# keeffEoghan/tendrils

Hardware: AMD Instinct MI355X
Metric: particle-steps/sec (16M particles per GPU) (higher is better)
Workload: dtype f32

## Files before the change

include/tendrils_hip.h:

```cpp
#ifndef TENDRILS_HIP_H
#define TENDRILS_HIP_H

#include <stddef.h>
#include <stdint.h>

#ifdef __cplusplus
extern "C" {
#endif

#define TH_ABI_VERSION 14

typedef int32_t th_status;
enum {
    TH_OK = 0,
    TH_ERR_INVALID = 1,
    TH_ERR_HIP = 2,
    TH_ERR_NO_DEVICE = 3,
    TH_ERR_UNSUPPORTED = 4
};

#define TH_INERT (-1000000.0f)

typedef struct th_context th_context;

// ... 295 lines not shown
    uint64_t fragments, crowded_fragments;
    uint64_t sent_bytes, received_bytes;
} th_draw_info;
th_status th_draw_query(th_context *ctx, th_draw_info *out);

typedef struct th_flow_line_uniforms {
    float speed, rad, crestShape, speedLimit;
    float viewSize[2];
} th_flow_line_uniforms;

th_status th_flow_line_attributes(const float *points, const double *times, int32_t n, int32_t closed, int32_t capacity,
                                  int32_t *nverts, float *position, float *normal, float *miter, float *previous,
                                  float *time, float *dt);
th_status th_flow_lines(th_context *ctx, const th_flow_line_uniforms *u, const float *points, const double *times,
                        const int32_t *offsets, const int32_t *closed, int32_t nlines);

enum { TH_OPT_BUCKET = 0, TH_OPT_RESORT_STEPS = 1, TH_OPT_REBUCKET_STEPS = 2, TH_OPT_FUSE = 3, TH_OPT_GRAPH = 4,
       TH_OPT_FORCE_GENERIC = 5, TH_OPT_DRAW_REUSE = 6, TH_OPT_BINS_POOL = 7,
#ifdef TH_TESTING
       TH_OPT_INJECT_FAILURE = 8,
#endif
       TH_OPT_BINS_PAGES = 9, TH_OPT_ASYNC_SORT = 10, TH_OPT_SKIP_UNSEEN = 11, TH_OPT_SPAWN_CHUNK_ROWS = 12,
       TH_OPT_HASH_WINDOW = 13, TH_OPT_HASH_WINDOW_LAUNCHES = 14, TH_OPT_DENSE_SORTS = 15,
       TH_OPT_STAGE_BINS = 16, TH_OPT_LINE_BINS = 17 };
th_status th_option_set(th_context *ctx, int32_t option, int64_t value);
th_status th_option_get(th_context *ctx, int32_t option, int64_t *value);

#ifdef __cplusplus
}
#endif
#endif
```

tendrils_amd/csrc/th_api.hip:

```cpp
#include "th_ctx.hpp"

using namespace thi;

namespace {

thread_local std::string g_error;

void build_gradient_table(float4 *lut)
{
    for (int a = th::kLutMin; a <= th::kLutMax; ++a) {
        float p = th::permute_ref((float)a);
        float gx, gy, gz;
        th::gradient_ref(p, gx, gy, gz);
        lut[a - th::kLutMin] = make_float4(gx, gy, gz, 0.0f);
    }
}

void options_from_environment(th_options &o)
{
    auto number = [](const char *name, long long otherwise) { const char *e = getenv(name); return e && *e ? atoll(e) : otherwise; };
    o.bucket = (int)number("TH_BUCKET", -1);
    o.resort_steps = (int)number("TH_RESORT_STEPS", 64); if (o.resort_steps <= 0) o.resort_steps = 64;
    o.rebucket_steps = (int)number("TH_REBUCKET_STEPS", 256); if (o.rebucket_steps <= 0) o.rebucket_steps = 256;
    o.fuse = number("TH_FUSE", 1) != 0;
// ... 521 lines not shown
    out->state_w = c->cfg.width; out->state_h = c->cfg.height;
    out->flow_w = c->fw; out->flow_h = c->fh;
    out->frames_w = c->frw; out->frames_h = c->frh;
    return TH_OK;
}

th_status th_option_set(th_context *c, int32_t option, int64_t value)
{
    if (th_status s = use(c)) return s;
    th_options &o = c->opt;
    switch (option) {
    case TH_OPT_BUCKET: TH_REQUIRE(value >= -1 && value <= 1, "TH_OPT_BUCKET takes -1, 0 or 1"); o.bucket = (int)value; break;
    case TH_OPT_RESORT_STEPS: TH_REQUIRE(value > 0 && value < (1 << 30), "TH_OPT_RESORT_STEPS must be positive"); o.resort_steps = (int)value; break;
    case TH_OPT_REBUCKET_STEPS: TH_REQUIRE(value > 0 && value < (1 << 30), "TH_OPT_REBUCKET_STEPS must be positive"); o.rebucket_steps = (int)value; break;
    case TH_OPT_FUSE: o.fuse = value != 0; break;
    case TH_OPT_GRAPH: o.graph = value != 0; break;
    case TH_OPT_FORCE_GENERIC: o.force_generic = value != 0; break;
    case TH_OPT_DRAW_REUSE: o.draw_reuse = value != 0; break;
    case TH_OPT_SKIP_UNSEEN: o.skip_unseen = value != 0; break;
    case TH_OPT_HASH_WINDOW: o.hash_window = value != 0; break;
    case TH_OPT_STAGE_BINS: o.stage_bins = value != 0; break;
    case TH_OPT_LINE_BINS: o.line_bins = value != 0; break;
    case TH_OPT_HASH_WINDOW_LAUNCHES: return fail(TH_ERR_INVALID, "TH_OPT_HASH_WINDOW_LAUNCHES is read-only");
    case TH_OPT_DENSE_SORTS: return fail(TH_ERR_INVALID, "TH_OPT_DENSE_SORTS is read-only");
    case TH_OPT_ASYNC_SORT: o.async_sort = value != 0; if (!o.async_sort) { if (th_status s = asort_drop(c)) return s; } break;
    case TH_OPT_BINS_POOL: TH_REQUIRE(value >= 0 && value < (1ll << 32), "TH_OPT_BINS_POOL out of range"); o.bins_pool = (uint32_t)value; break;
#ifdef TH_TESTING
    case TH_OPT_INJECT_FAILURE: TH_REQUIRE(value >= 0 && value <= 5, "TH_OPT_INJECT_FAILURE takes 0..5"); o.inject_failure = (int)value; break;
#endif
    case TH_OPT_SPAWN_CHUNK_ROWS: TH_REQUIRE(value >= 0 && value < (1 << 30), "TH_OPT_SPAWN_CHUNK_ROWS takes 0 (by the scratch budget) or a number of rows"); o.spawn_chunk_rows = (int)value; break;
    case TH_OPT_BINS_PAGES:
        TH_REQUIRE(value >= -(int64_t)th::kBinPagesLimit && value <= (int64_t)th::kBinPagesLimit && value != 1 && value != -1, "TH_OPT_BINS_PAGES takes 0, or 2..%u (negative: never widened)", th::kBinPagesLimit);
        o.bins_pages = (int)value;
        if (c->chunk_table) {
            TH_HIP(hipStreamSynchronize(c->stream));
            c->chunk_table.reset(); c->bin_mem.reset(); c->bin_capacity = 0; c->bin_max_pages = 0;
        }
        break;
    default: return fail(TH_ERR_INVALID, "unknown option %d", option);
    }
    clear_graphs(c);
    return TH_OK;
}

th_status th_option_get(th_context *c, int32_t option, int64_t *value)
{
    TH_REQUIRE(c && value, "null argument");
    const th_options &o = c->opt;
    switch (option) {
    case TH_OPT_BUCKET: *value = o.bucket; break;
    case TH_OPT_RESORT_STEPS: *value = o.resort_steps; break;
    case TH_OPT_REBUCKET_STEPS: *value = o.rebucket_steps; break;
    case TH_OPT_FUSE: *value = o.fuse; break;
    case TH_OPT_GRAPH: *value = o.graph; break;
    case TH_OPT_FORCE_GENERIC: *value = o.force_generic; break;
    case TH_OPT_DRAW_REUSE: *value = o.draw_reuse; break;
    case TH_OPT_ASYNC_SORT: *value = o.async_sort; break;
    case TH_OPT_SKIP_UNSEEN: *value = o.skip_unseen; break;
    case TH_OPT_HASH_WINDOW: *value = o.hash_window; break;
    case TH_OPT_STAGE_BINS: *value = o.stage_bins; break;
    case TH_OPT_LINE_BINS: *value = o.line_bins; break;
    case TH_OPT_HASH_WINDOW_LAUNCHES: *value = c->hash_window_launches; break;
    case TH_OPT_DENSE_SORTS: *value = c->dense_sorts; break;
    case TH_OPT_BINS_POOL: *value = o.bins_pool; break;
#ifdef TH_TESTING
    case TH_OPT_INJECT_FAILURE: *value = o.inject_failure; break;
#endif
    case TH_OPT_BINS_PAGES: *value = o.bins_pages; break;
    case TH_OPT_SPAWN_CHUNK_ROWS: *value = o.spawn_chunk_rows; break;
    default: return fail(TH_ERR_INVALID, "unknown option %d", option);
    }
    return TH_OK;
}

}
```

tendrils_amd/csrc/th_ctx.hpp:

```cpp
#pragma once
#include <hip/hip_runtime.h>

#include <algorithm>
#include <atomic>
#include <cmath>
#include <cstdarg>
#include <cstdio>
#include <cstdlib>
#include <cstring>
#include <limits>
#include <memory>
#include <mutex>
#include <new>
#include <string>
#include <vector>

#include "th_kernels.hpp"
#include "th_math.hpp"
#include "th_program_kinds.hpp"

namespace thi {
struct FlowLineScratch;
th_status fail(th_status code, const char *fmt, ...);
std::string &last_error();
// ... 84 lines not shown
    th::LogicParams key{};
    hipGraphExec_t exec = nullptr;
    DevBuf<float> times_dev;
    HostBuf<float> times_host;
    hipEvent_t copied = nullptr;
};

struct th_context {
    th_config cfg{};
    th_options opt{};
    hipStream_t stream = nullptr;
    std::vector<float4 *> ring;
    bool packed = false;
    DevBuf<float4> tmp[3];
    DevBuf<float4> flow;
    DevBuf<float2> flow_dec;
    DevBuf<float> flow3;
    int32_t fw = 0, fh = 0;
    DevBuf<float4> targets;
    bool targets_checked = true, targets_nonfinite = false;
    DevBuf<float4> lut_block;
    float4 *lut = nullptr;
    DevBuf<float4> win_block;
    long long dense_sorts = 0;
    long long hash_window_launches = 0;
    DevBuf<uchar4> frames[2];
    int32_t frw = 0, frh = 0;
    DevBuf<unsigned int> d_flag;
    DevBuf<th::StatsPartial> partials;
    DevBuf<th::StatsPartial> fused_parts;
    struct { bool valid = false; const float4 *buf = nullptr; float limit = 0.0f; uint32_t nparts = 0; } fused_stats;
    DevBuf<th_counters> d_counters;
    DevBuf<float4> x_halo;
    DevBuf<unsigned long long> x_counts;
    DevBuf<unsigned long long> x_keys;
    DevBuf<float4> x_colors;
    DevBuf<float4> gathered;
    const void *gathered_of = nullptr;
    DevBuf<char> sp_taps;
    DevBuf<uint32_t> sp_asked;
    DevBuf<float4> sp_answers;
    DevBuf<unsigned long long> sp_words;
    th_spawn_info last_spawn{};
    void *comm = nullptr;
    const th::Transport *transport = nullptr;
    DevBuf<uint32_t> d_status;
    DevBuf<uint32_t> own_mem;
    bool sharded_draw_ready = false;
// ... 302 lines not shown
```

tendrils_amd/csrc/th_kernels.hip:

```cpp
#include "th_kernels.hpp"
#include "th_math.hpp"
#include "th_logic.hpp"

#include <type_traits>
#include <cstdlib>

namespace th {


__global__ __launch_bounds__(256) void pack_state_kernel(uint2 *dst, const float4 *src, uint32_t n)
{
    for (uint32_t i = blockIdx.x * 256u + threadIdx.x; i < n; i += gridDim.x * 256u) dst[i] = pack_state(src[i]);
}

__global__ __launch_bounds__(256) void unpack_state_kernel(float4 *dst, const uint2 *src, uint32_t n)
{
    for (uint32_t i = blockIdx.x * 256u + threadIdx.x; i < n; i += gridDim.x * 256u) dst[i] = unpack_state(src[i]);
}

void launch_pack_state(void *dst, const float4 *src, uint32_t n, hipStream_t s)
{
    if (n) hipLaunchKernelGGL(pack_state_kernel, dim3(grid_for(n, 8)), dim3(256), 0, s, (uint2 *)dst, src, n);
}

void launch_unpack_state(float4 *dst, const void *src, uint32_t n, hipStream_t s)
{
    if (n) hipLaunchKernelGGL(unpack_state_kernel, dim3(grid_for(n, 8)), dim3(256), 0, s, dst, (const uint2 *)src, n);
}

__global__ __launch_bounds__(256) void hash_tables_kernel(float4 *block)
{
    uint32_t *a = reinterpret_cast<uint32_t *>(block), *b = a + kPermA;
    for (int k = threadIdx.x; k < kPermA; k += 256) a[k] = 4u * (uint32_t)permute_int((float)k) - kBiasBitsA;
    for (int k = threadIdx.x; k < kPermB; k += 256) b[k] = 16u * (uint32_t)((int)permute_int((float)k) - kLutMin) - kBiasBitsB;
}
void launch_hash_tables(float4 *block, hipStream_t s) { hipLaunchKernelGGL(hash_tables_kernel, dim3(1), dim3(256), 0, s, block); }
int hash_table_vectors() { return kHashVec; }

__global__ __launch_bounds__(256) void win_tables_kernel(float4 *block, const float4 *lut)
{
    uint32_t *a = reinterpret_cast<uint32_t *>(block), *b = a + kWinA;
    float4 *g = block + kWinVec;
    for (int k = threadIdx.x; k < kWinA; k += 256) a[k] = 4u * (uint32_t)permute_int((float)(k % 289)) - kBiasBitsA;
    for (int k = threadIdx.x; k < kWinB; k += 256) b[k] = 16u * (uint32_t)((int)permute_int((float)(k % 289)) - kLutMin) - kBiasBitsB;
    for (int k = threadIdx.x; k < kWinG; k += 256) g[k] = lut[k % 289 - kLutMin];
}
void launch_win_tables(float4 *block, const float4 *lut, hipStream_t s) { hipLaunchKernelGGL(win_tables_kernel, dim3(1), dim3(256), 0, s, block, lut); }
int win_table_vectors() { return kWinVec + kWinG; }



struct F32Texel {
    using Word = float4;
    static constexpr bool packed = false;
    TH_D static Word empty() { return make_float4(0.0f, 0.0f, 0.0f, 0.0f); }
    TH_D static Word load(const float4 *buf, uint32_t i) { return load_stream(&buf[i]); }
    TH_D static void store(float4 *buf, uint32_t i, Word w) { store_stream(&buf[i], w); }
    TH_D static float4 decode(Word w) { return w; }
    TH_D static Word encode(float4 s) { return s; }
    TH_D static float4 quantize(float4 s) { return s; }
};
struct PackedTexel {
    using Word = v2u;
    static constexpr bool packed = true;
    TH_D static Word empty() { return Word{0x80008000u, 0u}; }
    TH_D static Word load(const float4 *buf, uint32_t i) { return __builtin_nontemporal_load(&reinterpret_cast<const v2u *>(buf)[i]); }
    TH_D static void store(float4 *buf, uint32_t i, Word w) { __builtin_nontemporal_store(w, &reinterpret_cast<v2u *>(buf)[i]); }
    TH_D static float4 decode(Word w) { return unpack_state(make_uint2(w.x, w.y)); }
    TH_D static Word encode(float4 s) { const uint2 q = pack_state(s); return Word{q.x, q.y}; }
    TH_D static float4 quantize(float4 s) { return quantize_state(s); }
};
// ... 87 lines not shown
    double sum = fin ? (double)sp : 0.0;
    float mx = fin ? sp : 0.0f;
#pragma unroll
    for (int o = 32; o > 0; o >>= 1) {
        sum += __shfl_xor(sum, o);
        const float om = __shfl_xor(mx, o); mx = om > mx ? om : mx;
    }
    if (__lane_id() == (uint32_t)__builtin_ctzll(__ballot(true))) {
        t.sum_speed = sum; t.max_speed = (double)mx;
        if (!first) {
            const StatsPartial o = *slot;
            t.live += o.live; t.nan += o.nan; t.capped += o.capped; t.sum_speed += o.sum_speed;
            t.max_speed = o.max_speed > t.max_speed ? o.max_speed : t.max_speed;
        }
        *slot = t;
    }
}

TH_D void stats_none(StatsPartial *slot, bool first)
{
    if (__ballot(!first) == 0ull && __lane_id() == 0u) *slot = StatsPartial{0ull, 0ull, 0ull, 0.0, 0.0};
}

#define TH_LOGIC_FUSED_LOOP(Fmt)                                                                                              \
    static_assert(!WIN || (NOISE && !FAST), "WIN: NOISE, exact");                                                              \
    __shared__ float4 smem[WIN ? kWinVec + kWinG : NOISE ? kHashVec + kLutSize : 1];                                          \
    const float4 *lut = smem + (WIN ? kWinVec + kLutMin : NOISE ? kHashVec : 0);                                              \
    const HashTables tabs{reinterpret_cast<const uint32_t *>(smem), reinterpret_cast<const uint32_t *>(smem) + (WIN ? kWinA : kPermA)}; \
    if constexpr (NOISE) {                                                                                                    \
        if constexpr (WIN) fill_win_tables(smem, p.win);                                                                      \
        else fill_hash_tables(smem, p.lut);                                                                                   \
        __syncthreads();                                                                                                      \
    }                                                                                                                         \
    uint32_t idx, stride, end;                                                                                                \
    if constexpr (!BUCKETED) {                                                                                                \
        idx = blockIdx.x * 256u + threadIdx.x;                                                                                \
        stride = gridDim.x * 256u;                                                                                            \
        end = p.count;                                                                                                        \
    } else {                                                                                                                  \
        const uint32_t group = blockIdx.x & 7u, rank = blockIdx.x >> 3, per = (p.count + 7u) >> 3;                            \
        const uint32_t lo = group * per;                                                                                      \
        idx = lo + rank * 256u + threadIdx.x;                                                                                 \
        stride = (gridDim.x >> 3) * 256u;                                                                                     \
        end = lo + per < p.count ? lo + per : p.count;                                                                        \
    }                                                                                                                         \
    typename Fmt::Word nxt = Fmt::empty();                                                                                    \
    uint32_t npid = idx;                                                                                                      \
    [[maybe_unused]] bool first = true;                                                                                       \
    if (idx < end) {                                                                                                          \
        nxt = Fmt::load(p.in, idx);                                                                                           \
        if constexpr (BUCKETED) npid = __builtin_nontemporal_load(&p.perm[idx]);                                              \
    }                                                                                                                         \
    for (; idx < end; idx += stride) {                                                                                        \
        const typename Fmt::Word w = nxt;                                                                                     \
        const uint32_t pid = BUCKETED ? npid : idx;                                                                           \
        if (idx + stride < end) {                                                                                             \
            nxt = Fmt::load(p.in, idx + stride);                                                                              \
            if constexpr (BUCKETED) npid = __builtin_nontemporal_load(&p.perm[idx + stride]);                                 \
        }                                                                                                                     \
        float4 st = Fmt::decode(w);                                                                                           \
        uint32_t left = p.nsteps;                                                                                             \
        do {                                                                                                                  \
            if (left == 1u) {                                                                                                 \
                uint32_t at = idx;                                                                                            \
                asm volatile("" : "+v"(at));                                                                                  \
                if (Fmt::packed && p.nsteps == 1u) Fmt::store(p.out_prev, at, w);                                             \
                else Fmt::store(p.out_prev, at, Fmt::encode(st));                                                             \
            }                                                                                                                 \
            st = Fmt::quantize(integrate<FAST, NOISE, TARGET, POW2, false, true, !NOISE, WIN>(p, lut, st, pid, p.times[p.nsteps - left], &tabs)); \
        } while (--left);                                                                                                     \
        Fmt::store(p.out, idx, Fmt::encode(st));                                                                              \
        if constexpr (STATS) { stats_take(&p.stats_part[blockIdx.x * 4u + (threadIdx.x >> 6)], st, p.u.speedLimit, first); first = false; } \
    }                                                                                                                         \
    if constexpr (STATS) stats_none(&p.stats_part[blockIdx.x * 4u + (threadIdx.x >> 6)], first);

template <bool FAST, bool NOISE, bool TARGET, bool POW2, bool BUCKETED, bool STATS, bool WIN>
__global__ __launch_bounds__(256) void logic_fused_kernel(const LogicParams p) { TH_LOGIC_FUSED_LOOP(F32Texel) }

template <bool FAST, bool NOISE, bool TARGET, bool POW2, bool BUCKETED, bool STATS, bool WIN>
__global__ __launch_bounds__(256, 5) void logic_fused_packed_kernel(const LogicParams p) { TH_LOGIC_FUSED_LOOP(PackedTexel) }

int fused_grid(uint32_t count, bool bucketed)
{
    const uint32_t blocks = (count + 255u) / 256u;
    const uint32_t grid = bucketed ? 8u * ((((count + 7u) >> 3) + 255u) / 256u) : blocks;
    return (int)(grid ? grid : 1u);
}

void launch_logic_fused(const LogicParams &p, const LogicVariant &v, hipStream_t s)
{
    if (!p.nsteps) return;
    const bool packed = v.format == StateFormat::packed, bucketed = p.perm != nullptr;
    const int grid = fused_grid(p.count, bucketed);
    lift([&](auto fast, auto noise, auto target, auto pow2, auto bk, auto stats, auto window) {
        constexpr bool win = noise && !fast && window;
        hipLaunchKernelGGL((packed ? logic_fused_packed_kernel<fast, noise, target, pow2, bk, stats, win>
                                   : logic_fused_kernel<fast, noise, target, pow2, bk, stats, win>), dim3(grid), dim3(256), 0, s, p);
    }, v.mode == TH_MODE_FAST, v.noise, v.target, v.pow2, bucketed, p.stats_part != nullptr, p.win != nullptr);
}

// ... 1066 lines not shown
```

tendrils_amd/csrc/th_kernels.hpp:

```cpp
#pragma once
#include <string>

#include <hip/hip_runtime.h>
#include <stdint.h>

#include "../../include/tendrils_hip.h"

namespace th {

inline int grid_for(size_t n, int blocks_per_cu)
{
    size_t blocks = (n + 255) / 256;
    size_t cap = (size_t)256 * blocks_per_cu;
    return (int)(blocks < cap ? (blocks ? blocks : 1) : cap);
}

constexpr uint32_t kMaxFusedSteps = 32;
constexpr int kWinSpan = 286;
constexpr int kWinMaxCell = 8958;

constexpr uint32_t kTileChunk = 4096;
constexpr uint32_t kMaxTileBins = 8192;
constexpr uint32_t kDenseTileBins = 4096;
constexpr uint32_t kSortReplicas = 64;
constexpr uint32_t kBinSlotsLog2 = 6, kBinSlots = 1u << kBinSlotsLog2;

struct TileGeom {
    float view_x, view_y, half_fw, half_fh, fwm1, fhm1;
    uint32_t tiles_x, ntiles;
    uint32_t width, log2w, pow2w, row0;
    const uint32_t *row_draws;
};

struct TileChunk { uint32_t start, count, tile, pad; };
inline bool tile_sort_dense(const TileGeom &g) { return 2u * g.ntiles + 2u <= kDenseTileBins; }
struct ChunkRecord { uint32_t key[kBinSlots], count[kBinSlots]; };

struct LogicParams {
    const float4 *in;
    float4 *out;
    const float4 *flow;
    const float2 *flow_dec;
// ... 10 lines not shown
    float fwf, fhf, fwm1, fhm1, half_fw, half_fh;
    th_logic_uniforms u;
    float s2_cap;
    float pos_bound;
    const uint32_t *perm;
    TileGeom geom;
    const TileChunk *chunks;
    const uint32_t *nchunks;
    uint32_t *cursor;
    uint32_t *perm_out;
    float4 *in_moved;
    uint32_t *hist;
    ChunkRecord *records;
    uint32_t use_records;
    const float *time_dev;
    uint8_t *seen;
    float seen_xlo, seen_xhi, seen_ylo, seen_yhi;
    float4 *out_prev;
    uint32_t nsteps;
    struct StatsPartial *stats_part;
    float times[kMaxFusedSteps];
    const float4 *win;
    float win_bound;
    float win_k[2][3];
};

struct TileSortParams {
    const float4 *state;
    const uint32_t *perm_in;
    uint32_t count;
    TileGeom g;
    uint32_t *hist;
    uint32_t *cursor;
    uint32_t *totals, *starts;
    TileChunk *chunks;
    uint32_t *nchunks;
    float4 *state_out;
    uint32_t *perm_out;
    ChunkRecord *block_records;
    uint32_t packed;
};

struct OpticalFlowParams {
    const uchar4 *view, *last;
    float4 *flow;
    int32_t fr_w, fr_h;
    int32_t out_w, out_h;
// ... 153 lines not shown
    resort,
    count_in_place,
};

void launch_logic(const LogicParams &p, const LogicVariant &v, hipStream_t stream);
void launch_logic_generic(const LogicParams &p, hipStream_t stream);
void launch_logic_fused(const LogicParams &p, const LogicVariant &v, hipStream_t stream);
inline bool fused_taps_flow3(const LogicVariant &v) { return !v.noise; }
void launch_pack_state(void *dst, const float4 *src, uint32_t n, hipStream_t stream);
void launch_unpack_state(float4 *dst, const void *src, uint32_t n, hipStream_t stream);
void launch_flow_pack3(const float4 *flow, float *xyz, size_t n, hipStream_t stream);
void launch_flow_decode(const float4 *flow, float2 *dec, size_t n, float time, const float *time_dev, float decay,
                        hipStream_t stream);
void launch_logic_sorted(const LogicParams &p, const LogicVariant &v, SortedPass pass, uint32_t max_chunks, hipStream_t stream);
void launch_tile_hist(const TileSortParams &b, hipStream_t stream);
void launch_tile_scan(const TileSortParams &b, hipStream_t stream);
void launch_tile_scatter(const TileSortParams &b, hipStream_t stream);
void launch_unpermute_state(float4 *dst, const float4 *src, const uint32_t *perm, uint32_t n, bool packed, hipStream_t stream);
void launch_permute_state(float4 *dst, const float4 *src, const uint32_t *perm, uint32_t n, bool packed, hipStream_t stream);
void launch_fill(float4 *dst, float4 value, size_t n, hipStream_t stream);
void launch_hash_tables(float4 *block, hipStream_t stream);
int hash_table_vectors();
void launch_win_tables(float4 *block, const float4 *lut, hipStream_t stream);
int win_table_vectors();
void launch_finite_check(const float4 *src, size_t n, unsigned int *flag, hipStream_t stream);
void launch_stats_fold(const StatsPartial *parts, uint32_t nparts, StatsPartial *scratch, size_t n, const unsigned long long *respawned,
                       th_counters *out, hipStream_t stream);
uint32_t fused_stats_parts(uint32_t count, bool sorted);
int fused_grid(uint32_t count, bool bucketed);
void launch_stats(const float4 *state, size_t n, float speed_limit, StatsPartial *partials, const unsigned long long *respawned,
                  th_counters *out, hipStream_t stream);
void launch_counter_add(unsigned long long *counter, unsigned long long n, hipStream_t s);
void launch_optical_flow(const OpticalFlowParams &p, hipStream_t stream);
uint32_t deposit_scan_words(uint32_t W, uint32_t rows);
size_t deposit_list_words(uint32_t W, uint32_t rows, uint32_t *cap);
void launch_deposit_count(const DepositParams &p, hipStream_t stream);
void launch_deposit_scan(const DepositParams &p, uint32_t *scratch, uint32_t *total, hipStream_t stream);
void launch_deposit_scatter(const DepositParams &p, hipStream_t stream);
struct alignas(16) FragmentLine { uint32_t line; float along, across, length; };
void launch_fragment_lines(const DepositParams &p, FragmentLine *lines, hipStream_t stream);
void launch_fragment_line_ends(const DepositParams &p, int4 *ends, hipStream_t stream, bool program);
void launch_fragment_lines_bins(const DepositParams &p, const int4 *ends, FragmentLine *lines, int deal, hipStream_t stream);
constexpr int kBinsStageDeal = 2, kBinsStageDealCrowded = 8;
int deposit_key_bits(const DepositParams &p);
void launch_export_mark(const DepositParams &p, hipStream_t stream);
void launch_export_write(const DepositParams &p, float *out, hipStream_t stream);
// ... 79 lines not shown
```

tendrils_amd/csrc/th_logic.hpp:

```cpp
#pragma once
#include "th_kernels.hpp"
#include "th_math.hpp"

namespace th {

typedef float v4f __attribute__((ext_vector_type(4)));
typedef unsigned v2u __attribute__((ext_vector_type(2)));
typedef float v2f __attribute__((ext_vector_type(2)));

TH_D uint32_t mad_u24_s(uint32_t a, uint32_t b, uint32_t c)
{
    uint32_t r;
    asm("v_mad_u32_u24 %0, %1, %2, %3" : "=v"(r) : "v"(a), "s"(b), "v"(c));
    return r;
}

TH_D float4 load_stream(const float4 *p)
{
    v4f v = __builtin_nontemporal_load(reinterpret_cast<const v4f *>(p));
    return make_float4(v.x, v.y, v.z, v.w);
}
TH_D void store_stream(float4 *p, float4 a)
{
    v4f v = {a.x, a.y, a.z, a.w};
// ... 44 lines not shown
    nvx *= r; nvy *= r;
    return make_float4(posx + nvx, posy + nvy, nvx, nvy);
}

struct NoiseCorners {
    float ax, ay, az, bx, by, bz, cx, cy, cz, dx, dy, dz;
    int j0, j1, j2, j3;
};

constexpr uint32_t kBiasBitsA = 0x4A000000u, kBiasBitsB = 0x49000000u;
constexpr int kPermA = 292, kPermB = 584;
constexpr int kHashVec = (kPermA + kPermB) / 4;
struct HashTables {
    const uint32_t *permA, *permB;
};

TH_D void fill_hash_tables(float4 *smem, const float4 *lut_global)
{
    const float4 *block = lut_global - kHashVec;
    for (int k = threadIdx.x; k < kHashVec + kLutSize; k += 256) smem[k] = block[k];
}

constexpr int kWinA = 580, kWinB = 868, kWinG = 868;
constexpr int kWinVec = (kWinA + kWinB) / 4;
static_assert(288 + kWinSpan + 2 < kWinA && 2 * 288 + kWinSpan + 1 < kWinB, "i - c <= 288 + kWinSpan (th_kernels.hpp) stays inside the tables");

TH_D void fill_win_tables(float4 *smem, const float4 *win_global)
{
    for (int k = threadIdx.x; k < kWinVec + kWinG; k += 256) smem[k] = win_global[k];
}


template <bool FAST, bool WIN = false>
TH_D NoiseCorners snoise_corners_tab(float vx, float vy, float vz, float sxy, const HashTables &T, const float *K = nullptr)
{
    NoiseCorners n;
    float s = mad<FAST>(vz, kC3, sxy);
    float ix = th_floor(vx + s), iy = th_floor(vy + s), iz = th_floor(vz + s);
    float t = mad<FAST>(iz, kC6, mad<FAST>(iy, kC6, ix * kC6));
    float ax = (vx - ix) + t, ay = (vy - iy) + t, az = (vz - iz) + t;

    const float ax1 = ax - 1.0f, ay1 = ay - 1.0f, az1 = az - 1.0f;
    float bx, by, bz, cx, cy, cz;
    uint32_t e1x, e2x;
    unsigned long long my1, my2, mz1, mz2;
    {
        unsigned long long l1, l2, l3, m;
        asm("v_cmp_lt_f32 %[l1], %[ax], %[ay]\n\t"
            "v_cmp_lt_f32 %[l2], %[ay], %[az]\n\t"
            "v_cmp_lt_f32 %[l3], %[az], %[ax]\n\t"
            "s_andn2_b64 %[m], %[l3], %[l1]\n\t"     "v_cndmask_b32 %[bx], %[ax], %[ax1], %[m]\n\t"   "v_cndmask_b32 %[e1x], 0, 16, %[m]\n\t"
            "s_andn2_b64 %[my1], %[l1], %[l2]\n\t"   "v_cndmask_b32 %[by], %[ay], %[ay1], %[my1]\n\t"
            "s_andn2_b64 %[mz1], %[l2], %[l3]\n\t"   "v_cndmask_b32 %[bz], %[az], %[az1], %[mz1]\n\t"
            "s_orn2_b64 %[m], %[l3], %[l1]\n\t"      "v_cndmask_b32 %[cx], %[ax], %[ax1], %[m]\n\t"   "v_cndmask_b32 %[e2x], 0, 16, %[m]\n\t"
            "s_orn2_b64 %[my2], %[l1], %[l2]\n\t"    "v_cndmask_b32 %[cy], %[ay], %[ay1], %[my2]\n\t"
            "s_orn2_b64 %[mz2], %[l2], %[l3]\n\t"    "v_cndmask_b32 %[cz], %[az], %[az1], %[mz2]"
            : [l1] "=&s"(l1), [l2] "=&s"(l2), [l3] "=&s"(l3), [m] "=&s"(m),
              [my1] "=&s"(my1), [my2] "=&s"(my2), [mz1] "=&s"(mz1), [mz2] "=&s"(mz2),
              [bx] "=&v"(bx), [by] "=&v"(by), [bz] "=&v"(bz), [cx] "=&v"(cx), [cy] "=&v"(cy), [cz] "=&v"(cz),
              [e1x] "=&v"(e1x), [e2x] "=&v"(e2x)
            : [ax] "v"(ax), [ay] "v"(ay), [az] "v"(az), [ax1] "v"(ax1), [ay1] "v"(ay1), [az1] "v"(az1)
            : "scc");
    }
    n.ax = ax; n.ay = ay; n.az = az;
    n.bx = bx + kC6; n.by = by + kC6; n.bz = bz + kC6;
    n.cx = cx + kC3; n.cy = cy + kC3; n.cz = cz + kC3;
    n.dx = ax - 0.5f; n.dy = ay - 0.5f; n.dz = az - 0.5f;

    uint32_t zb, yb, xb;
    if constexpr (WIN) {
        asm("v_add_f32_sdwa %0, %2, %1 dst_sel:WORD_0 dst_unused:UNUSED_PAD src0_sel:DWORD src1_sel:DWORD"
            : "=v"(zb) : "v"(iz), "s"(K[0]));
        asm("v_add_f32 %0, %2, %1" : "=v"(yb) : "v"(iy), "s"(K[1]));
        asm("v_add_f32 %0, %2, %1" : "=v"(xb) : "v"(ix), "s"(K[2]));
    } else {
        asm("v_add_f32 %0, 0x4a000000, %1" : "=v"(zb) : "v"(mod289_int(iz)));
        asm("v_add_f32 %0, 0x4a000000, %1" : "=v"(yb) : "v"(mod289_int(iy)));
        asm("v_add_f32 %0, 0x49000000, %1" : "=v"(xb) : "v"(mod289_int(ix)));
        zb &= 0xffcu;
    }
    const uint32_t *pa = reinterpret_cast<const uint32_t *>(reinterpret_cast<const char *>(T.permA) + zb);
    const uint32_t a0 = pa[0] + yb, a1 = pa[1] + yb;
    const uint32_t *pu = reinterpret_cast<const uint32_t *>(reinterpret_cast<const char *>(T.permB) + a0);
    const uint32_t *pw = reinterpret_cast<const uint32_t *>(reinterpret_cast<const char *>(T.permB) + a1);
    const uint32_t u0 = pu[0], u1 = pu[1], w0 = pw[0], w1 = pw[1];
    uint32_t q1, q2, t1, t2;
    asm("v_cndmask_b32 %0, %1, %2, %3" : "=v"(t1) : "v"(u0), "v"(u1), "s"(my1));
    asm("v_cndmask_b32 %0, %1, %2, %3" : "=v"(q1) : "v"(t1), "v"(w0), "s"(mz1));
    asm("v_cndmask_b32 %0, %1, %2, %3" : "=v"(t2) : "v"(w0), "v"(w1), "s"(my2));
    asm("v_cndmask_b32 %0, %1, %2, %3" : "=v"(q2) : "v"(u1), "v"(t2), "s"(mz2));
    n.j0 = (int)(u0 + xb); n.j1 = (int)(q1 + (xb + e1x)); n.j2 = (int)(q2 + (xb + e2x)); n.j3 = (int)(w1 + xb + 16u);
    return n;
}

TH_D float4 lut_at_offset(const float4 *lut, int off)
{
    return *reinterpret_cast<const float4 *>(reinterpret_cast<const char *>(lut) + off);
}

template <bool FAST>
TH_D NoiseCorners snoise_corners(float vx, float vy, float vz, float sxy)
{
    NoiseCorners n;
    float s = mad<FAST>(vz, kC3, sxy);
    float ix = th_floor(vx + s), iy = th_floor(vy + s), iz = th_floor(vz + s);
    float t = mad<FAST>(iz, kC6, mad<FAST>(iy, kC6, ix * kC6));
    float ax = (vx - ix) + t, ay = (vy - iy) + t, az = (vz - iz) + t;

// ... 115 lines not shown
    int ty = (int)__builtin_amdgcn_fmed3f((sy + 1.0f) * p.half_fh, 0.0f, p.fhm1);
    float ffx, ffy;
    float4 ft;
    if constexpr (DECODED) { float2 d = p.flow_dec[ty * p.fw + tx]; ffx = d.x; ffy = d.y; }
    else {
        const uint32_t texel = mad_u24_s((uint32_t)ty, (uint32_t)p.fw, (uint32_t)tx);
        if constexpr (FLOW3) {
            const float *f3 = reinterpret_cast<const float *>(reinterpret_cast<const char *>(p.flow3) + ((texel + (texel << 1)) << 2));
            ft = make_float4(f3[0], f3[1], f3[2], 0.0f);
        } else {
            ft = *reinterpret_cast<const float4 *>(reinterpret_cast<const char *>(p.flow) + (texel << 4));
        }
    }

    float wxs = 0.0f, wys = 0.0f;
    if constexpr (NOISE) {
        float nscale = vary(u.noiseScale, i, u.varyNoiseScale);
        float nx = posx * nscale, ny = posy * nscale;
        float ntime = time * vary(u.noiseSpeed, i, u.varyNoiseSpeed);
        float sxy = mad<FAST>(ny, kC3, nx * kC3);
        NoiseCorners na, nb;
        float4 a0, a1, a2, a3, b0, b1, b2, b3;
        if constexpr (PTAB) {
            na = snoise_corners_tab<FAST, WIN>(nx, ny, uvx + ntime, sxy, *tabs, p.win_k[0]);
            nb = snoise_corners_tab<FAST, WIN>(nx, ny, (uvy + ntime) + 1234.5678f, sxy, *tabs, p.win_k[1]);
            a0 = lut_at_offset(lut, na.j0); a1 = lut_at_offset(lut, na.j1); a2 = lut_at_offset(lut, na.j2); a3 = lut_at_offset(lut, na.j3);
            b0 = lut_at_offset(lut, nb.j0); b1 = lut_at_offset(lut, nb.j1); b2 = lut_at_offset(lut, nb.j2); b3 = lut_at_offset(lut, nb.j3);
        } else {
            na = snoise_corners<FAST>(nx, ny, uvx + ntime, sxy);
            nb = snoise_corners<FAST>(nx, ny, (uvy + ntime) + 1234.5678f, sxy);
            a0 = lut_at(lut, na.j0); a1 = lut_at(lut, na.j1); a2 = lut_at(lut, na.j2); a3 = lut_at(lut, na.j3);
            b0 = lut_at(lut, nb.j0); b1 = lut_at(lut, nb.j1); b2 = lut_at(lut, nb.j2); b3 = lut_at(lut, nb.j3);
        }
        float wx = snoise_finish<FAST>(na, a0, a1, a2, a3);
        float wy = snoise_finish<FAST>(nb, b0, b1, b2, b3);
        float vnw = vary(u.noiseWeight, i, u.varyNoise);
        wxs = (wx * u.dt) * vnw; wys = (wy * u.dt) * vnw;
    }

    if constexpr (!DECODED) {
        float k = __builtin_fmaxf(0.0f, 1.0f - ((time - ft.z) * u.flowDecay));
        ffx = ft.x * k; ffy = ft.y * k;
    }
    float vflw = vary(u.flowWeight, i, u.varyFlow);
    float fxs = (ffx * u.dt) * vflw, fys = (ffy * u.dt) * vflw;
    float vfw = vary(u.forceWeight, i, u.varyForce);
    float nvx, nvy;
    if constexpr (NOISE) {
// ... 30 lines not shown
```

tendrils_amd/csrc/th_step.hip:

```cpp
#include "th_ctx.hpp"

using namespace thi;

namespace {

float s2_cap_for(float limit)
{
    if (!(limit > 0.0f)) return -1.0f;
    if (std::isinf(limit)) return std::numeric_limits<float>::max();
    double sq = (double)limit * (double)limit;
    if (sq >= (double)std::numeric_limits<float>::max()) return std::numeric_limits<float>::max();
    float c = (float)sq;
    while (sqrtf(c) > limit) c = nextafterf(c, 0.0f);
    for (;;) {
        float n = nextafterf(c, std::numeric_limits<float>::infinity());
        if (std::isinf(n) || sqrtf(n) > limit) break;
        c = n;
    }
    return c;
}

bool finite_uniforms(const th_logic_uniforms &u)
{
    const float *f = reinterpret_cast<const float *>(&u);
    for (size_t k = 0; k < sizeof(u) / sizeof(float); ++k)
        if (!std::isfinite(f[k])) return false;
    return true;
}

constexpr double kWinNoiseUnits = 64.0;
constexpr double kWinMinViews = 2.0;
bool hash_window(const th_logic_uniforms &u, float pos_bound, const float *times, int32_t m, float *win_bound, float (*win_k)[3])
{
    const double N = kWinNoiseUnits;
    const double scale0 = u.noiseScale, scale1 = scale0 + (double)u.varyNoiseScale * scale0;
    const double scale = std::fmax(std::fabs(scale0), std::fabs(scale1));
    *win_bound = (float)(scale > 0.0 ? std::fmin((double)pos_bound, N / scale) : (double)pos_bound);
    if (!((double)*win_bound * std::fmin(std::fabs((double)u.viewSize[0]), std::fabs((double)u.viewSize[1])) >= kWinMinViews)) return false;
    const double speed0 = u.noiseSpeed, speed1 = speed0 + (double)u.varyNoiseSpeed * speed0;
    double tlo = std::numeric_limits<double>::infinity(), thi = -tlo;
    for (int32_t k = 0; k < m; ++k)
        for (double speed : {speed0, speed1}) {
            const double nt = (double)times[k] * speed;
            tlo = std::fmin(tlo, nt); thi = std::fmax(thi, nt);
        }
    for (int e = 0; e < 2; ++e) {
        const double zlo = tlo + (e ? 1234.5678 : 0.0), zhi = thi + 1.0 + (e ? 1234.5678 : 0.0);
        const double slo = zlo / 3.0 - 2.0 * N / 3.0, shi = zhi / 3.0 + 2.0 * N / 3.0;
        const double lo[2] = {std::floor(-N + slo) - 2.0, std::floor(zlo + slo) - 2.0};
        const double hi[2] = {std::floor(N + shi) + 2.0, std::floor(zhi + shi) + 2.0};
        double c[2];
        for (int a = 0; a < 2; ++a) {
            if (!(hi[a] - lo[a] <= (double)th::kWinSpan)) return false;
            if (!(std::fmax(std::fabs(lo[a]), std::fabs(hi[a])) + 1.0 <= (double)th::kWinMaxCell)) return false;
            c[a] = 289.0 * std::floor(lo[a] / 289.0);
        }
        win_k[e][0] = (float)(2097152.0 - c[1]);
        win_k[e][1] = (float)(2097152.0 - c[0]);
        win_k[e][2] = (float)(524288.0 - c[0]);
    }
    return true;
}

}

struct StepPlan {
    th::LogicParams p{};
    th::LogicVariant v;
    bool generic = false;
    bool may_sort = false;
};

static th_status plan_step(th_context *c, const th_logic_uniforms &u, int32_t target, StepPlan &plan)
{
    const uint32_t W = (uint32_t)c->cfg.width, H = (uint32_t)c->cfg.global_height;
    th::LogicParams &p = plan.p;
    p = th::LogicParams{};
    p.flow = c->flow; p.flow_dec = c->flow_dec; p.targets = c->targets; p.lut = c->lut;
    p.count = (uint32_t)c->texels();
    p.width = W;
    p.row0 = (uint32_t)c->cfg.row0;
    p.wf = (float)W; p.hf = (float)H;
// ... 245 lines not shown
    return step_done(c, packed_kernel, target, p, s);
}

static th_status step_n_fused(th_context *c, const StepPlan &plan, const std::vector<float> &times, int32_t n)
{
    if (th_status s = fused_slots(c, plan.may_sort, tile_geom(c, plan.p.u))) return s;
    const bool pack3 = th::fused_taps_flow3(plan.v);
    if (pack3) {
        if (!c->flow3) if (th_status s = c->flow3.alloc((size_t)c->fw * c->fh * 3)) return s;
        th::launch_flow_pack3(c->flow, c->flow3, (size_t)c->fw * c->fh, c->stream);
    }
    for (int32_t done = 0; done < n;) {
        const int32_t m = std::min<int32_t>(n - done, (int32_t)th::kMaxFusedSteps);
        th::LogicParams p = plan.p;
        p.flow3 = pack3 ? c->flow3 : nullptr;
        const int order = order_of(c, c->ring[0]);
        const FusedRoute r = fused_route(c, m);
        p.in = r.in;
        p.out = r.out;
        p.out_prev = r.out_prev;
        p.perm = order >= 0 ? c->orders[(size_t)order].perm : nullptr;
        p.nsteps = (uint32_t)m;
        for (int32_t k = 0; k < m; ++k) p.times[k] = times[(size_t)(done + k)];
        const bool window = plan.v.noise && plan.v.mode != TH_MODE_FAST && c->opt.hash_window && hash_window(p.u, p.pos_bound, p.times, m, &p.win_bound, p.win_k);
        if (window) p.win = c->win_block;
        const bool takes_stats = done + m == n;
        if (takes_stats) {
            const uint32_t parts = th::fused_stats_parts(p.count, p.perm != nullptr), need = parts + (parts + 255u) / 256u + 16u;
            if (c->fused_parts.size() < need) {
                TH_HIP(hipStreamSynchronize(c->stream));
                if (th_status s = c->fused_parts.alloc(need)) return s;
            }
            p.stats_part = c->fused_parts;
            c->fused_stats.nparts = parts; c->fused_stats.limit = p.u.speedLimit;
        }
        LaunchTimer timer;
        if (th_status s = timer.begin(c)) return s;
        th::launch_logic_fused(p, plan.v, c->stream);
        if (th_status s = timer.end(c)) return s;
        TH_HIP(hipGetLastError());
        if (window) ++c->hash_window_launches;
        set_order(c, r.other, order);
        c->counted.buf = nullptr;
        fused_routed(c, m);
        done += m;
        if (takes_stats) { c->fused_stats.valid = true; c->fused_stats.buf = c->ring[0]; }
    }
    return TH_OK;
// ... 100 lines not shown
```

tendrils_amd/particles.py:

```python
import ctypes as C

import numpy as np

from . import _capi
from ._capi import call


def defaults():
    return dict(shape=[64, 64], geomShape=None,
                logic=None, logicVert=None, logicFrag=None,
                render=None, renderVert=None, renderFrag=None)


class Program:

    COMPILE, SOURCE_KIND = "th_program_compile", "user"

    def __init__(self, kind, **fixed):
        self.kind = kind
        self.fixed = fixed
        self.uniforms = {}
        self.handle = None
        self.uniforms_struct = None

# ... 315 lines not shown
            call("th_step_program_view_size", self._ctx, None)
        else:
            call("th_step_program_view_size", self._ctx, (C.c_float * 2)(float(view_size[0]), float(view_size[1])))

    def draw(self, update=None, mode=None):
        return None

    def updateLogic(self, logicFrag):
        self.logic = logicFrag if isinstance(logicFrag, Program) else Program(LOGIC)

    def updateRender(self, *a):
        pass

    def sync(self):
        call("th_sync", self._ctx)

    def draw_pipeline(self, which):
        call("th_draw_pipeline", self._ctx, {"auto": -1, "stream": 0, "bins": 1}[which])

    OPTIONS = dict(bucket=0, resort_steps=1, rebucket_steps=2, fuse=3, graph=4, force_generic=5, draw_reuse=6, bins_pool=7,
                   inject_failure=8, bins_pages=9, async_sort=10, skip_unseen=11, spawn_chunk_rows=12,
                   hash_window=13, hash_window_launches=14, dense_sorts=15, stage_bins=16)
    MORE_OPTIONS = dict(line_bins=17)

    @classmethod
    def option_number(cls, name):
        return cls.OPTIONS[name] if name in cls.OPTIONS else cls.MORE_OPTIONS[name]

    def option(self, name, value=None):
        number = self.option_number(name)
        if value is not None:
            call("th_option_set", self._ctx, number, int(value))
        out = C.c_int64(0)
        call("th_option_get", self._ctx, number, C.byref(out))
        return out.value

    def fetches_taps(self, source):
        if self.sharded_spawn != "auto":
            return bool(self.sharded_spawn)
        if source < 0 or self._global_height in (0, self.shape[1]):
            return False
        q = _capi.CommInfo()
        call("th_comm_query", self._ctx, C.byref(q))
        return bool(q.active)

    def deposit_flow(self, view_size, time, speed_limit):
        u = deposit_uniforms(view_size, time, speed_limit)
        n = C.c_uint64(0)
        call("th_flow_deposit", self._ctx, C.byref(u), C.byref(n))
        return int(n.value)
# ... 165 lines not shown
```

Baseline: 221.6 billion.

## Merge window hash tables into gradient LUT and precompute skew products per window origin

Restructures the windowed noise hash tables: permutation offsets are packed into the w lane of the gradient LUT, and a new table of precomputed (cell+origin)*C6 products replaces the three-multiply skew sum with three shared-memory loads indexed by the same SDWA-computed offsets. The products table is refilled by a small kernel only when the window origins change, with a counter exposed as a read-only option. It also raises launch bounds to 6 waves for the windowed non-target kernel and adds a guard that rejects windows whose z range straddles zero. The goal is less ALU and shared-memory footprint per noise evaluation, at the cost of extra LDS loads, more register pressure under the tighter occupancy bound, and added host-side state tracking.

```diff
diff --git a/include/tendrils_hip.h b/include/tendrils_hip.h
--- a/include/tendrils_hip.h
+++ b/include/tendrils_hip.h
@@ -341,7 +341,7 @@
 #endif
        TH_OPT_BINS_PAGES = 9, TH_OPT_ASYNC_SORT = 10, TH_OPT_SKIP_UNSEEN = 11, TH_OPT_SPAWN_CHUNK_ROWS = 12,
        TH_OPT_HASH_WINDOW = 13, TH_OPT_HASH_WINDOW_LAUNCHES = 14, TH_OPT_DENSE_SORTS = 15,
-       TH_OPT_STAGE_BINS = 16, TH_OPT_LINE_BINS = 17 };
+       TH_OPT_STAGE_BINS = 16, TH_OPT_LINE_BINS = 17, TH_OPT_HASH_WINDOW_REFILLS = 18 };
 th_status th_option_set(th_context *ctx, int32_t option, int64_t value);
 th_status th_option_get(th_context *ctx, int32_t option, int64_t *value);
 
diff --git a/tendrils_amd/csrc/th_api.hip b/tendrils_amd/csrc/th_api.hip
--- a/tendrils_amd/csrc/th_api.hip
+++ b/tendrils_amd/csrc/th_api.hip
@@ -567,6 +567,7 @@
     case TH_OPT_STAGE_BINS: o.stage_bins = value != 0; break;
     case TH_OPT_LINE_BINS: o.line_bins = value != 0; break;
     case TH_OPT_HASH_WINDOW_LAUNCHES: return fail(TH_ERR_INVALID, "TH_OPT_HASH_WINDOW_LAUNCHES is read-only");
+    case TH_OPT_HASH_WINDOW_REFILLS: return fail(TH_ERR_INVALID, "TH_OPT_HASH_WINDOW_REFILLS is read-only");
     case TH_OPT_DENSE_SORTS: return fail(TH_ERR_INVALID, "TH_OPT_DENSE_SORTS is read-only");
     case TH_OPT_ASYNC_SORT: o.async_sort = value != 0; if (!o.async_sort) { if (th_status s = asort_drop(c)) return s; } break;
     case TH_OPT_BINS_POOL: TH_REQUIRE(value >= 0 && value < (1ll << 32), "TH_OPT_BINS_POOL out of range"); o.bins_pool = (uint32_t)value; break;
@@ -606,6 +607,7 @@
     case TH_OPT_STAGE_BINS: *value = o.stage_bins; break;
     case TH_OPT_LINE_BINS: *value = o.line_bins; break;
     case TH_OPT_HASH_WINDOW_LAUNCHES: *value = c->hash_window_launches; break;
+    case TH_OPT_HASH_WINDOW_REFILLS: *value = c->hash_window_refills; break;
     case TH_OPT_DENSE_SORTS: *value = c->dense_sorts; break;
     case TH_OPT_BINS_POOL: *value = o.bins_pool; break;
 #ifdef TH_TESTING
diff --git a/tendrils_amd/csrc/th_ctx.hpp b/tendrils_amd/csrc/th_ctx.hpp
--- a/tendrils_amd/csrc/th_ctx.hpp
+++ b/tendrils_amd/csrc/th_ctx.hpp
@@ -130,8 +130,11 @@
     DevBuf<float4> lut_block;
     float4 *lut = nullptr;
     DevBuf<float4> win_block;
+    th::WinOrigins win_origins{};
+    bool win_origins_valid = false;
     long long dense_sorts = 0;
     long long hash_window_launches = 0;
+    long long hash_window_refills = 0;
     DevBuf<uchar4> frames[2];
     int32_t frw = 0, frh = 0;
     DevBuf<unsigned int> d_flag;
diff --git a/tendrils_amd/csrc/th_kernels.hip b/tendrils_amd/csrc/th_kernels.hip
--- a/tendrils_amd/csrc/th_kernels.hip
+++ b/tendrils_amd/csrc/th_kernels.hip
@@ -39,14 +39,22 @@
 
 __global__ __launch_bounds__(256) void win_tables_kernel(float4 *block, const float4 *lut)
 {
-    uint32_t *a = reinterpret_cast<uint32_t *>(block), *b = a + kWinA;
-    float4 *g = block + kWinVec;
-    for (int k = threadIdx.x; k < kWinA; k += 256) a[k] = 4u * (uint32_t)permute_int((float)(k % 289)) - kBiasBitsA;
-    for (int k = threadIdx.x; k < kWinB; k += 256) b[k] = 16u * (uint32_t)((int)permute_int((float)(k % 289)) - kLutMin) - kBiasBitsB;
-    for (int k = threadIdx.x; k < kWinG; k += 256) g[k] = lut[k % 289 - kLutMin];
+    for (int k = threadIdx.x; k < kWinG; k += 256) {
+        float4 g = lut[k % 289 - kLutMin];
+        g.w = __uint_as_float(16u * (uint32_t)permute_int((float)(k % 289)));
+        block[k] = g;
+    }
+    for (int k = threadIdx.x; k < kWinT; k += 256) block[kWinG + k] = make_float4(0.0f, 0.0f, 0.0f, 0.0f);
 }
 void launch_win_tables(float4 *block, const float4 *lut, hipStream_t s) { hipLaunchKernelGGL(win_tables_kernel, dim3(1), dim3(256), 0, s, block, lut); }
-int win_table_vectors() { return kWinVec + kWinG; }
+int win_table_vectors() { return kWinG + kWinT; }
+
+__global__ __launch_bounds__(256) void win_products_kernel(float4 *block, WinOrigins c)
+{
+    for (int k = threadIdx.x; k < kWinT; k += 256)
+        block[kWinG + k] = make_float4((float)(k + c.c[0]) * kC6, (float)(k + c.c[1]) * kC6, (float)(k + c.c[2]) * kC6, (float)(k + c.c[3]) * kC6);
+}
+void launch_win_products(float4 *block, const WinOrigins &c, hipStream_t s) { hipLaunchKernelGGL(win_products_kernel, dim3(1), dim3(256), 0, s, block, c); }
 
 
 
@@ -180,11 +188,26 @@
     if (__ballot(!first) == 0ull && __lane_id() == 0u) *slot = StatsPartial{0ull, 0ull, 0ull, 0.0, 0.0};
 }
 
+template <bool LATE>
+TH_D StatsPartial *stats_slot(const LogicParams &p)
+{
+    uint32_t wave = threadIdx.x >> 6;
+    if constexpr (LATE) asm volatile("" : "+v"(wave));
+    return &p.stats_part[blockIdx.x * 4u + wave];
+}
+template <bool LATE>
+TH_D float stats_limit(const LogicParams &p)
+{
+    float limit = p.u.speedLimit;
+    if constexpr (LATE) asm volatile("" : "+s"(limit));
+    return limit;
+}
+
 #define TH_LOGIC_FUSED_LOOP(Fmt)                                                                                              \
     static_assert(!WIN || (NOISE && !FAST), "WIN: NOISE, exact");                                                              \
-    __shared__ float4 smem[WIN ? kWinVec + kWinG : NOISE ? kHashVec + kLutSize : 1];                                          \
-    const float4 *lut = smem + (WIN ? kWinVec + kLutMin : NOISE ? kHashVec : 0);                                              \
-    const HashTables tabs{reinterpret_cast<const uint32_t *>(smem), reinterpret_cast<const uint32_t *>(smem) + (WIN ? kWinA : kPermA)}; \
+    __shared__ float4 smem[WIN ? kWinG + kWinT : NOISE ? kHashVec + kLutSize : 1];                                            \
+    const float4 *lut = smem + (!WIN && NOISE ? kHashVec : 0);                                                                \
+    const HashTables tabs{reinterpret_cast<const uint32_t *>(smem) + (WIN ? 3 : 0), reinterpret_cast<const uint32_t *>(smem) + (WIN ? 3 : kPermA)}; \
     if constexpr (NOISE) {                                                                                                    \
         if constexpr (WIN) fill_win_tables(smem, p.win);                                                                      \
         else fill_hash_tables(smem, p.lut);                                                                                   \
@@ -228,12 +251,12 @@
             st = Fmt::quantize(integrate<FAST, NOISE, TARGET, POW2, false, true, !NOISE, WIN>(p, lut, st, pid, p.times[p.nsteps - left], &tabs)); \
         } while (--left);                                                                                                     \
         Fmt::store(p.out, idx, Fmt::encode(st));                                                                              \
-        if constexpr (STATS) { stats_take(&p.stats_part[blockIdx.x * 4u + (threadIdx.x >> 6)], st, p.u.speedLimit, first); first = false; } \
+        if constexpr (STATS) { stats_take(stats_slot<WIN>(p), st, stats_limit<WIN>(p), first); first = false; }               \
     }                                                                                                                         \
-    if constexpr (STATS) stats_none(&p.stats_part[blockIdx.x * 4u + (threadIdx.x >> 6)], first);
+    if constexpr (STATS) stats_none(stats_slot<WIN>(p), first);
 
 template <bool FAST, bool NOISE, bool TARGET, bool POW2, bool BUCKETED, bool STATS, bool WIN>
-__global__ __launch_bounds__(256) void logic_fused_kernel(const LogicParams p) { TH_LOGIC_FUSED_LOOP(F32Texel) }
+__global__ __launch_bounds__(256, WIN && !TARGET ? 6 : 1) void logic_fused_kernel(const LogicParams p) { TH_LOGIC_FUSED_LOOP(F32Texel) }
 
 template <bool FAST, bool NOISE, bool TARGET, bool POW2, bool BUCKETED, bool STATS, bool WIN>
 __global__ __launch_bounds__(256, 5) void logic_fused_packed_kernel(const LogicParams p) { TH_LOGIC_FUSED_LOOP(PackedTexel) }
diff --git a/tendrils_amd/csrc/th_kernels.hpp b/tendrils_amd/csrc/th_kernels.hpp
--- a/tendrils_amd/csrc/th_kernels.hpp
+++ b/tendrils_amd/csrc/th_kernels.hpp
@@ -18,6 +18,7 @@
 constexpr uint32_t kMaxFusedSteps = 32;
 constexpr int kWinSpan = 286;
 constexpr int kWinMaxCell = 8958;
+constexpr double kWinMinZ = 1.0 / 1024.0;
 
 constexpr uint32_t kTileChunk = 4096;
 constexpr uint32_t kMaxTileBins = 8192;
@@ -74,7 +75,12 @@
     float times[kMaxFusedSteps];
     const float4 *win;
     float win_bound;
-    float win_k[2][3];
+    float win_k[2][2];
+};
+
+struct WinOrigins {
+    int32_t c[4];
+    bool operator==(const WinOrigins &o) const { return c[0] == o.c[0] && c[1] == o.c[1] && c[2] == o.c[2] && c[3] == o.c[3]; }
 };
 
 struct TileSortParams {
@@ -274,6 +280,7 @@
 void launch_hash_tables(float4 *block, hipStream_t stream);
 int hash_table_vectors();
 void launch_win_tables(float4 *block, const float4 *lut, hipStream_t stream);
+void launch_win_products(float4 *block, const WinOrigins &c, hipStream_t stream);
 int win_table_vectors();
 void launch_finite_check(const float4 *src, size_t n, unsigned int *flag, hipStream_t stream);
 void launch_stats_fold(const StatsPartial *parts, uint32_t nparts, StatsPartial *scratch, size_t n, const unsigned long long *respawned,
diff --git a/tendrils_amd/csrc/th_logic.hpp b/tendrils_amd/csrc/th_logic.hpp
--- a/tendrils_amd/csrc/th_logic.hpp
+++ b/tendrils_amd/csrc/th_logic.hpp
@@ -90,22 +90,37 @@
 }
 
 constexpr int kWinA = 580, kWinB = 868, kWinG = 868;
-constexpr int kWinVec = (kWinA + kWinB) / 4;
-static_assert(288 + kWinSpan + 2 < kWinA && 2 * 288 + kWinSpan + 1 < kWinB, "i - c <= 288 + kWinSpan (th_kernels.hpp) stays inside the tables");
+constexpr int kWinT = 576;
+static_assert(288 + kWinSpan + 2 < kWinA && 2 * 288 + kWinSpan + 1 < kWinB && kWinA <= kWinG && kWinB <= kWinG && 288 + kWinSpan < kWinT,
+              "i - c <= 288 + kWinSpan (th_kernels.hpp) stays inside the tables");
+static_assert(16 * (kWinG - 1) < 1 << 16, "every offset fits the half word the bias adds write");
 
 TH_D void fill_win_tables(float4 *smem, const float4 *win_global)
 {
-    for (int k = threadIdx.x; k < kWinVec + kWinG; k += 256) smem[k] = win_global[k];
-}
-
-
-template <bool FAST, bool WIN = false>
+    for (int k = threadIdx.x; k < kWinG + kWinT; k += 256) smem[k] = win_global[k];
+}
+
+
+template <bool FAST, bool WIN = false, int E = 0>
 TH_D NoiseCorners snoise_corners_tab(float vx, float vy, float vz, float sxy, const HashTables &T, const float *K = nullptr)
 {
     NoiseCorners n;
     float s = mad<FAST>(vz, kC3, sxy);
     float ix = th_floor(vx + s), iy = th_floor(vy + s), iz = th_floor(vz + s);
-    float t = mad<FAST>(iz, kC6, mad<FAST>(iy, kC6, ix * kC6));
+    uint32_t zb, yb, xb;
+    float t;
+    if constexpr (WIN) {
+        asm("v_add_f32_sdwa %0, %6, %3 dst_sel:WORD_0 dst_unused:UNUSED_PAD src0_sel:DWORD src1_sel:DWORD\n\t"
+            "v_add_f32_sdwa %1, %6, %4 dst_sel:WORD_0 dst_unused:UNUSED_PAD src0_sel:DWORD src1_sel:DWORD\n\t"
+            "v_add_f32_sdwa %2, %7, %5 dst_sel:WORD_0 dst_unused:UNUSED_PAD src0_sel:DWORD src1_sel:DWORD"
+            : "=&v"(yb), "=&v"(xb), "=&v"(zb) : "v"(iy), "v"(ix), "v"(iz), "s"(K[1]), "s"(K[0]));
+        const char *prod = reinterpret_cast<const char *>(T.permA) - 12 + 16 * kWinG + 4 * E;
+        const float z6 = *reinterpret_cast<const float *>(prod + 8 + zb);
+        const float y6 = *reinterpret_cast<const float *>(prod + yb), x6 = *reinterpret_cast<const float *>(prod + xb);
+        t = z6 + (y6 + x6);
+    } else {
+        t = mad<FAST>(iz, kC6, mad<FAST>(iy, kC6, ix * kC6));
+    }
     float ax = (vx - ix) + t, ay = (vy - iy) + t, az = (vz - iz) + t;
 
     const float ax1 = ax - 1.0f, ay1 = ay - 1.0f, az1 = az - 1.0f;
@@ -135,23 +150,18 @@
     n.cx = cx + kC3; n.cy = cy + kC3; n.cz = cz + kC3;
     n.dx = ax - 0.5f; n.dy = ay - 0.5f; n.dz = az - 0.5f;
 
-    uint32_t zb, yb, xb;
-    if constexpr (WIN) {
-        asm("v_add_f32_sdwa %0, %2, %1 dst_sel:WORD_0 dst_unused:UNUSED_PAD src0_sel:DWORD src1_sel:DWORD"
-            : "=v"(zb) : "v"(iz), "s"(K[0]));
-        asm("v_add_f32 %0, %2, %1" : "=v"(yb) : "v"(iy), "s"(K[1]));
-        asm("v_add_f32 %0, %2, %1" : "=v"(xb) : "v"(ix), "s"(K[2]));
-    } else {
+    constexpr int kNext = WIN ? 4 : 1;
+    if constexpr (!WIN) {
         asm("v_add_f32 %0, 0x4a000000, %1" : "=v"(zb) : "v"(mod289_int(iz)));
         asm("v_add_f32 %0, 0x4a000000, %1" : "=v"(yb) : "v"(mod289_int(iy)));
         asm("v_add_f32 %0, 0x49000000, %1" : "=v"(xb) : "v"(mod289_int(ix)));
         zb &= 0xffcu;
     }
     const uint32_t *pa = reinterpret_cast<const uint32_t *>(reinterpret_cast<const char *>(T.permA) + zb);
-    const uint32_t a0 = pa[0] + yb, a1 = pa[1] + yb;
+    const uint32_t a0 = pa[0] + yb, a1 = pa[kNext] + yb;
     const uint32_t *pu = reinterpret_cast<const uint32_t *>(reinterpret_cast<const char *>(T.permB) + a0);
     const uint32_t *pw = reinterpret_cast<const uint32_t *>(reinterpret_cast<const char *>(T.permB) + a1);
-    const uint32_t u0 = pu[0], u1 = pu[1], w0 = pw[0], w1 = pw[1];
+    const uint32_t u0 = pu[0], u1 = pu[kNext], w0 = pw[0], w1 = pw[kNext];
     uint32_t q1, q2, t1, t2;
     asm("v_cndmask_b32 %0, %1, %2, %3" : "=v"(t1) : "v"(u0), "v"(u1), "s"(my1));
     asm("v_cndmask_b32 %0, %1, %2, %3" : "=v"(q1) : "v"(t1), "v"(w0), "s"(mz1));
@@ -313,8 +323,8 @@
         NoiseCorners na, nb;
         float4 a0, a1, a2, a3, b0, b1, b2, b3;
         if constexpr (PTAB) {
-            na = snoise_corners_tab<FAST, WIN>(nx, ny, uvx + ntime, sxy, *tabs, p.win_k[0]);
-            nb = snoise_corners_tab<FAST, WIN>(nx, ny, (uvy + ntime) + 1234.5678f, sxy, *tabs, p.win_k[1]);
+            na = snoise_corners_tab<FAST, WIN, 0>(nx, ny, uvx + ntime, sxy, *tabs, p.win_k[0]);
+            nb = snoise_corners_tab<FAST, WIN, 1>(nx, ny, (uvy + ntime) + 1234.5678f, sxy, *tabs, p.win_k[1]);
             a0 = lut_at_offset(lut, na.j0); a1 = lut_at_offset(lut, na.j1); a2 = lut_at_offset(lut, na.j2); a3 = lut_at_offset(lut, na.j3);
             b0 = lut_at_offset(lut, nb.j0); b1 = lut_at_offset(lut, nb.j1); b2 = lut_at_offset(lut, nb.j2); b3 = lut_at_offset(lut, nb.j3);
         } else {
diff --git a/tendrils_amd/csrc/th_step.hip b/tendrils_amd/csrc/th_step.hip
--- a/tendrils_amd/csrc/th_step.hip
+++ b/tendrils_amd/csrc/th_step.hip
@@ -30,7 +30,7 @@
 
 constexpr double kWinNoiseUnits = 64.0;
 constexpr double kWinMinViews = 2.0;
-bool hash_window(const th_logic_uniforms &u, float pos_bound, const float *times, int32_t m, float *win_bound, float (*win_k)[3])
+bool hash_window(const th_logic_uniforms &u, float pos_bound, const float *times, int32_t m, float *win_bound, float (*win_k)[2], th::WinOrigins *origins)
 {
     const double N = kWinNoiseUnits;
     const double scale0 = u.noiseScale, scale1 = scale0 + (double)u.varyNoiseScale * scale0;
@@ -46,6 +46,7 @@
         }
     for (int e = 0; e < 2; ++e) {
         const double zlo = tlo + (e ? 1234.5678 : 0.0), zhi = thi + 1.0 + (e ? 1234.5678 : 0.0);
+        if (!(zlo >= th::kWinMinZ || zhi <= -th::kWinMinZ)) return false;
         const double slo = zlo / 3.0 - 2.0 * N / 3.0, shi = zhi / 3.0 + 2.0 * N / 3.0;
         const double lo[2] = {std::floor(-N + slo) - 2.0, std::floor(zlo + slo) - 2.0};
         const double hi[2] = {std::floor(N + shi) + 2.0, std::floor(zhi + shi) + 2.0};
@@ -55,9 +56,10 @@
             if (!(std::fmax(std::fabs(lo[a]), std::fabs(hi[a])) + 1.0 <= (double)th::kWinMaxCell)) return false;
             c[a] = 289.0 * std::floor(lo[a] / 289.0);
         }
-        win_k[e][0] = (float)(2097152.0 - c[1]);
-        win_k[e][1] = (float)(2097152.0 - c[0]);
-        win_k[e][2] = (float)(524288.0 - c[0]);
+        win_k[e][0] = (float)(524288.0 - c[1]);
+        win_k[e][1] = (float)(524288.0 - c[0]);
+        origins->c[e] = (int32_t)c[0];
+        origins->c[2 + e] = (int32_t)c[1];
     }
     return true;
 }
@@ -349,8 +351,17 @@
         p.perm = order >= 0 ? c->orders[(size_t)order].perm : nullptr;
         p.nsteps = (uint32_t)m;
         for (int32_t k = 0; k < m; ++k) p.times[k] = times[(size_t)(done + k)];
-        const bool window = plan.v.noise && plan.v.mode != TH_MODE_FAST && c->opt.hash_window && hash_window(p.u, p.pos_bound, p.times, m, &p.win_bound, p.win_k);
-        if (window) p.win = c->win_block;
+        th::WinOrigins origins;
+        const bool window = plan.v.noise && plan.v.mode != TH_MODE_FAST && c->opt.hash_window && hash_window(p.u, p.pos_bound, p.times, m, &p.win_bound, p.win_k, &origins);
+        if (window) {
+            p.win = c->win_block;
+            if (!c->win_origins_valid || !(c->win_origins == origins)) {
+                th::launch_win_products(c->win_block, origins, c->stream);
+                c->win_origins = origins;
+                c->win_origins_valid = true;
+                ++c->hash_window_refills;
+            }
+        }
         const bool takes_stats = done + m == n;
         if (takes_stats) {
             const uint32_t parts = th::fused_stats_parts(p.count, p.perm != nullptr), need = parts + (parts + 255u) / 256u + 16u;
diff --git a/tendrils_amd/particles.py b/tendrils_amd/particles.py
--- a/tendrils_amd/particles.py
+++ b/tendrils_amd/particles.py
@@ -361,10 +361,14 @@
                    inject_failure=8, bins_pages=9, async_sort=10, skip_unseen=11, spawn_chunk_rows=12,
                    hash_window=13, hash_window_launches=14, dense_sorts=15, stage_bins=16)
     MORE_OPTIONS = dict(line_bins=17)
+    LATER_OPTIONS = dict(hash_window_refills=18)
 
     @classmethod
     def option_number(cls, name):
-        return cls.OPTIONS[name] if name in cls.OPTIONS else cls.MORE_OPTIONS[name]
+        for table in (cls.OPTIONS, cls.MORE_OPTIONS):
+            if name in table:
+                return table[name]
+        return cls.LATER_OPTIONS[name]
 
     def option(self, name, value=None):
         number = self.option_number(name)
```

Result: no change. 219.8 billion (-0.8%).
